# inferflow/inferflow

Measured on AMD Instinct MI355X. Metric: decode tokens/sec, Llama-2-7B Q4 batch=1 greedy (whole job), higher is better.
Workload: dtype i8 (Q8 activations x Q4_B32T1A weights, i32 dot, f32 scale, f16 I/O); 1 GPU; llama2_7b decode, Q4_B32T1A weights + F16 lm_head, F16 KV cache, batch 1 greedy, 16-token prompt, context 21..1851; parallelism=single, weights_bytes=4309647360

## Files before the change

### include/inferflow_amd.h

```cpp
#ifndef INFERFLOW_AMD_H_
#define INFERFLOW_AMD_H_

#include <stddef.h>
#include <stdint.h>

#ifdef __cplusplus
extern "C" {
#endif

typedef enum {
    IFA_F32 = 0, IFA_F16 = 1,
    IFA_Q8_B32T1 = 7, IFA_Q8_B32T2 = 8, IFA_Q6_B64T1 = 9, IFA_Q5_B64T1 = 10, IFA_Q5_B32T1 = 11,
    IFA_Q4_B16 = 12, IFA_Q4_B32T1A = 13, IFA_Q4_B32T1B = 14, IFA_Q4_B64T1 = 17, IFA_Q3H_B64T1 = 18,
    IFA_Q3_B32T1A = 19, IFA_Q3_B32T1B = 20, IFA_Q2_B32T1A = 21, IFA_Q2_B32T1B = 22
} ifa_dtype;

enum {
    IFA_OK = 0,
    IFA_ERR_ARG = -1,
    IFA_ERR_DTYPE = -2,
    IFA_ERR_HIP = -3,
    IFA_ERR_STATE = -4,
    IFA_ERR_NOMEM = -5
};
// ... 227 lines not shown
    int vocab_offset;
    int force_collectives;
} ifa_tp_topology;
int ifa_model_tp_decode(ifa_model *m, const ifa_tp_topology *topo, int first_token, int start_pos, int n_steps,
                        int *out_tokens_host, float *elapsed_ms);
int ifa_model_tp_prefill(ifa_model *m, const ifa_tp_topology *topo, const int *tokens_host, int n_tokens, int start_pos,
                         void *logits_shard_out_dev, int *next_token_host);
int ifa_model_tp_decode_batch(ifa_model *m, const ifa_tp_topology *topo, int n, const int *tokens_host, const int *positions_host,
                              const int *kv_slots_host, int *next_tokens_host, void *logits_shard_out_dev);
int ifa_model_get_tensor(ifa_model *m, int layer, int tensor_id, int *dtype, void **dptr, size_t *rows, size_t *cols);
int ifa_model_get_expert_tensor(ifa_model *m, int layer, int expert, int tensor_id, int *dtype, void **dptr, size_t *rows, size_t *cols);
int ifa_model_time_kernel(ifa_model *m, int which, int iters, float *avg_us);

int ifa_decode_route_plan(const int *facts, int n_facts, int *out, int n_out);
int ifa_model_decode_route(ifa_model *m, int *out, int n_out);

int ifa_prompt_route_plan(const int *facts, int n_facts, int *out, int n_out);
int ifa_batch_route_plan(const int *facts, int n_facts, int *out, int n_out);
int ifa_model_prompt_route(ifa_model *m, int *out, int n_out);

#ifdef __cplusplus
}
#endif
#endif
```

### inferflow_amd/_capi.py

```python
import ctypes as C
import os

_HERE = os.path.dirname(os.path.abspath(__file__))
_LIB_PATH = os.environ.get("IFA_LIB") or os.path.join(_HERE, "lib", "libinferflow_amd.so")
_lib = None


class IfaError(RuntimeError):
    def __init__(self, code, msg):
        super().__init__("inferflow_amd error %d: %s" % (code, msg))
        self.code = code


def library_path():
    return _LIB_PATH


def lib():
    global _lib
    if _lib is None:
        if not os.path.exists(_LIB_PATH):
            raise ImportError(
                "inferflow_amd: %s is missing -- run `python __graft_entry__.py build` "
                "(hipcc --offload-arch=gfx950); there is no CPU fallback" % _LIB_PATH)
# ... 96 lines not shown
    "ifa_model_decode_draft": (_i, [_vp, _i, _vp, _i, _vp, _vp]),
    "ifa_model_set_pool_excluded": (_i, [_vp, _vp, _i]),
    "ifa_model_decode_pool": (_i, [_vp, _i, _i, _i, _vp, _vp, _vp, _vp]),
    "ifa_model_decode_batch_pool": (_i, [_vp, _i, _vp, _vp, _vp, _vp, _i, _vp, _i, _vp, _vp, _vp]),
    "ifa_model_forward_pool": (_i, [_vp, _vp, _i, _i, _vp, _i, _vp, _vp, _vp, _vp]),
    "ifa_model_pool_lse": (_i, [_vp, _vp, _i, _vp]),
    "ifa_model_logit_state_reset": (_i, [_vp, _i, _vp, _i, _f, _f, _f, _vp, _vp, _i]),
    "ifa_model_logit_state_add": (_i, [_vp, _i, _vp, _vp]),
    "ifa_model_pool_adjust": (_i, [_vp, _i, _vp]),
    "ifa_model_forward_score": (_i, [_vp, _vp, _i, _i, _vp, _vp, _vp, _vp]),
    "ifa_model_get_buffer": (_i, [_vp, C.c_char_p, _i, C.POINTER(_vp), C.POINTER(_sz)]),
    "ifa_model_stream": (_vp, [_vp]),
    "ifa_model_time_kernel": (_i, [_vp, _i, _i, _vp]),
    "ifa_decode_route_plan": (_i, [_vp, _i, _vp, _i]),
    "ifa_model_decode_route": (_i, [_vp, _vp, _i]),
    "ifa_prompt_route_plan": (_i, [_vp, _i, _vp, _i]),
    "ifa_batch_route_plan": (_i, [_vp, _i, _vp, _i]),
    "ifa_model_prompt_route": (_i, [_vp, _vp, _i]),
    "ifa_model_set_stream": (_i, [_vp, _vp]),
    "ifa_model_tp_begin": (_i, [_vp, _i, _i]),
    "ifa_model_tp_begin_hidden": (_i, [_vp, _vp, _i]),
    "ifa_model_tp_hidden": (_i, [_vp, _vp]),
    "ifa_model_tp_attn": (_i, [_vp, _i, _vp]),
    "ifa_model_tp_post_attn": (_i, [_vp, _i, _vp]),
    "ifa_model_tp_ffn": (_i, [_vp, _i, _vp]),
    "ifa_model_tp_post_ffn": (_i, [_vp, _i, _vp]),
    "ifa_model_tp_logits": (_i, [_vp, _vp]),
    "ifa_model_tp_set_token": (_i, [_vp, _vp]),
    "ifa_comm_unique_id": (_i, [_vp]),
    "ifa_comm_init_rank": (_i, [_vp, _i, _i, _i, C.POINTER(_vp)]),
# ... 115 lines not shown
```

### inferflow_amd/csrc/ifa_decode_route.h

```cpp
#pragma once
#include <algorithm>
#include <cstddef>
#include <cstring>

static constexpr size_t IFA_LDS_LIMIT = 160 * 1024;

namespace ifa {
constexpr int DEC_ATTN_MAX_SPLITS = 32;
constexpr int DEC_PV_STAGE = 4096;

constexpr size_t dec_attn_scores_smem(int head_dim, bool q8) { return q8 ? 16 : (size_t)256 * (head_dim * 2 + 16); }
constexpr size_t dec_attn_pv_smem(int head_dim, int max_ctx, int nsplits = 8)
{
    const size_t nsplit = 256 / (head_dim / 8);
    const size_t chunk = (((size_t)max_ctx + nsplits - 1) / nsplits + 63) / 64 * 64;
    return 8 * 4 + nsplit * head_dim * 4 + (size_t)(DEC_PV_STAGE + 8) * 2 + chunk * 2 + 16;
}
constexpr size_t dec_attn_smem(int head_dim, int max_ctx, int ktile_rows = 0)
{
    const size_t nsplit = 256 / (head_dim / 8);
    return (size_t)head_dim * 3 * 2 + 16 * 4 + nsplit * head_dim * 4 + (size_t)ktile_rows * head_dim * 2 + (((size_t)max_ctx * 2 + 15) & ~(size_t)15) + 16;
}

inline bool dec_qkv_attn_ul_shape(int rw, int gk) { return (rw == 6 && gk == 8) || (rw == 3 && gk == 32); }
// ... 48 lines not shown
        r.kt = kt_fits;
        const bool unload = (f.attn_unload >= 1 && bucket == 256) || (f.attn_unload >= 2 && bucket == 128 && (r.kt || f.kv_q8));
        r.ul = unload && dec_qkv_attn_ul_shape(f.rw, f.gk);
        r.pb = (r.ul && bucket == 64) || (!f.kv_q8 && !r.kt) ? 256 : bucket;
        r.gk = f.gk; r.rw = f.rw;
    }
    if (r.kind != DEC_ROUTE_SPLIT) r.lds_attn = (int)dec_attn_smem(f.head_dim, f.max_ctx, r.kt ? r.pb : 0);
    if (!f.own_launches) {
        r.chain = (f.fuse_ffn && f.waits && f.num_cus <= f.visible_cus) ? std::min(f.fuse_ffn, 2) : 0;
        if (r.chain == 2 && (!f.have_attq || !f.attn_q8 || f.head_dim % 32 != 0)) r.chain = 1;
        r.chain = std::min(r.chain, f.chain_level);
    }
    return r;
}

}
```

### inferflow_amd/csrc/ifa_engine.hip

```cpp
#include <mutex>
#include <unordered_map>
#include "ifa_engine_state.h"

namespace ifa {

namespace {
struct SpaceBook {
    std::mutex mu;
    std::unordered_map<void *, size_t> live;
    long long live_bytes = 0, fail_at = 0;
};
SpaceBook &book() { static SpaceBook *b = new SpaceBook(); return *b; }

template <class Alloc> int space_alloc(const char *call, void **p, size_t bytes, Alloc alloc)
{
    SpaceBook &b = book();
    *p = nullptr;
    {
        std::lock_guard<std::mutex> g(b.mu);
        if (b.fail_at > 0 && --b.fail_at == 0)
            return ifa_fail(IFA_ERR_HIP, "%s(%zu bytes) failed: out of memory (simulated: ifa_debug_alloc_fail_at)", call, bytes);
    }
    const hipError_t e = alloc(p, bytes);
    if (e != hipSuccess) {
// ... 65 lines not shown

int perf_collect(ifa_model *m)
{
    if (m->perf_spans.empty()) return IFA_OK;
    IFA_HIP_CHECK(hipStreamSynchronize(m->stream));
    for (auto &r : m->perf_spans) {
        float ms = 0.0f;
        if (hipEventElapsedTime(&ms, r.e0, r.e1) == hipSuccess) m->perf_map[r.key] += ms;
        else (void)hipGetLastError();
        m->perf_pool.push_back(r.e0); m->perf_pool.push_back(r.e1);
    }
    m->perf_spans.clear();
    return IFA_OK;
}

void drop_graphs(ifa_model *m)
{
    if (m->tp_graph_exec) { (void)hipGraphExecDestroy(m->tp_graph_exec); m->tp_graph_exec = nullptr; }
    if (m->tp_graph) { (void)hipGraphDestroy(m->tp_graph); m->tp_graph = nullptr; }
    if (m->graph_exec) { (void)hipGraphExecDestroy(m->graph_exec); m->graph_exec = nullptr; }
    if (m->graph) { (void)hipGraphDestroy(m->graph); m->graph = nullptr; }
    if (m->graph_exec_n) { (void)hipGraphExecDestroy(m->graph_exec_n); m->graph_exec_n = nullptr; }
    if (m->graph_n) { (void)hipGraphDestroy(m->graph_n); m->graph_n = nullptr; }
    for (auto &sl : m->slots) {
        if (sl.exec) { (void)hipGraphExecDestroy(sl.exec); sl.exec = nullptr; }
        if (sl.graph) { (void)hipGraphDestroy(sl.graph); sl.graph = nullptr; }
    }
    for (auto &kv : m->batch_graphs) if (kv.second) (void)hipGraphExecDestroy(kv.second);
    m->batch_graphs.clear();
    for (auto &kv : m->draft_graphs) if (kv.second) (void)hipGraphExecDestroy(kv.second);
    m->draft_graphs.clear();
    sampled_drop_graphs(m);
}

int ensure_scratch(ifa_model *m, int T)
{
    if (T <= m->scratch_tokens) return IFA_OK;
    const ifa_model_config &c = m->cfg;
    const size_t D = c.dim, QD = (size_t)c.heads * c.head_dim, KVD = (size_t)c.kv_heads * c.head_dim, F = c.ffn;
    size_t maxcols = std::max(std::max(D, QD), F);
    Scratch n;
    int rc;
// ... 359 lines not shown
    IFA_HIP_CHECK(hipStreamSynchronize(m->stream));
    return IFA_OK;
}

int ifa_model_select_kv(ifa_model *m, int slot)
{
    IFA_REQUIRE(m && m->finalized, "ifa_model_select_kv: model not finalized");
    if (m->slots.empty()) m->slots.resize(1);
    IFA_REQUIRE(slot >= 0 && slot < (int)m->slots.size(), "ifa_model_select_kv: slot %d of %zu", slot, m->slots.size());
    if (slot == m->cur_slot) return IFA_OK;
    if (m->tp_graph_exec) { (void)hipGraphExecDestroy(m->tp_graph_exec); m->tp_graph_exec = nullptr; }
    if (m->tp_graph) { (void)hipGraphDestroy(m->tp_graph); m->tp_graph = nullptr; }
    ifa_model::KvSlot &out = m->slots[(size_t)m->cur_slot], &in = m->slots[(size_t)slot];
    out.k.clear(); out.v.clear();
    for (Layer &L : m->layers) { out.k.push_back(std::move(L.kcache)); out.v.push_back(std::move(L.vcache)); }
    out.graph = m->graph; out.exec = m->graph_exec;
    if (m->graph_exec_n) { (void)hipGraphExecDestroy(m->graph_exec_n); m->graph_exec_n = nullptr; }
    if (m->graph_n) { (void)hipGraphDestroy(m->graph_n); m->graph_n = nullptr; }
    for (size_t l = 0; l < m->layers.size(); l++) { m->layers[l].kcache = std::move(in.k[l]); m->layers[l].vcache = std::move(in.v[l]); }
    m->graph = in.graph; m->graph_exec = in.exec;
    in.k.clear(); in.v.clear(); in.graph = nullptr; in.exec = nullptr;
    m->cur_slot = slot;
    return IFA_OK;
}

int ifa_model_set_option(ifa_model *m, const char *name, int value)
{
    IFA_REQUIRE(m && name, "ifa_model_set_option: null pointer");
    if (strcmp(name, "pool_lse") == 0) { m->opt_pool_lse = value != 0; return IFA_OK; }
    struct { const char *n; int *p; } opts[] = {
        {"fused", &m->opt_fused}, {"graph", &m->opt_graph}, {"rpw_qkv", &m->opt_rpw_qkv}, {"rpw_wo", &m->opt_rpw_wo},
        {"rpw_ffn", &m->opt_rpw_ffn}, {"rpw_w2", &m->opt_rpw_w2}, {"rpw_lm", &m->opt_rpw_lm}, {"trace", &m->opt_trace},
        {"bench_mode", &m->opt_bench_mode}, {"touch_stride", &m->opt_touch_stride}, {"attn_split_ctx", &m->opt_attn_split_ctx}, {"batch_graph", &m->opt_batch_graph}, {"gemm_rows", &m->opt_gemm_rows}, {"batch_fused", &m->opt_batch_fused}, {"rows_mo", &m->opt_rows_mo}, {"debug_mo_alloc_fail", &m->opt_debug_mo_alloc_fail}, {"rows_kparts", &m->opt_rows_kparts}, {"prefill_chunk", &m->opt_prefill_chunk}, {"prefill_big_min", &m->opt_prefill_big_min}, {"prefill_mid", &m->opt_prefill_mid}, {"prefill_mid_max", &m->opt_prefill_mid_max}, {"prefill_res_mid", &m->opt_prefill_res_mid}, {"gemm_splitk", &m->opt_gemm_splitk}, {"moe_singles", &m->opt_moe_singles}, {"moe_overlap", &m->opt_moe_overlap}, {"prefill_big", &m->opt_prefill_big}, {"moe_router_fused", &m->opt_moe_router_fused}, {"tp_fuse_add", &m->opt_tp_fuse_add}, {"attn_q8", &m->opt_attn_q8}, {"attn_kt", &m->opt_attn_kt}, {"fuse_attn", &m->opt_fuse_attn}, {"fuse_ffn", &m->opt_fuse_ffn}, {"attn_post_as_residual", &m->opt_attn_post_as_residual}, {"chain_late_w2", &m->opt_chain_late_w2}, {"exact_order", &m->opt_exact_order}, {"perf_stat", &m->opt_perf_stat}, {"attn_nsplits", &m->opt_attn_nsplits}, {"attn_unload", &m->opt_attn_unload}, {"q3h_native", &m->opt_q3h_native}, {"fuse_attn_timeout_us", &m->opt_fuse_attn_timeout_us}, {"step_tail", &m->opt_step_tail}, {"graph_steps", &m->opt_graph_steps}, {"moe_device", &m->opt_moe_device}, 
        
        {"debug_layers", &m->opt_debug_layers}, {"debug_layer0", &m->opt_debug_layer0}, {"debug_hidden_in", &m->opt_debug_hidden_in}};
    for (auto &o : opts)
// ... 37 lines not shown
    IFA_REQUIRE(m, "ifa_model_fused_supported: null model");
    std::string w;
    bool ok = fused_supported(m, &w);
    if (why && why_len) { strncpy(why, w.c_str(), why_len - 1); why[why_len - 1] = 0; }
    return ok ? 1 : 0;
}

int ifa_decode_route_plan(const int *facts, int n_facts, int *out, int n_out)
{
    IFA_REQUIRE(facts && out && n_facts == DEC_ROUTE_N_FACTS && n_out >= DEC_ROUTE_N_OUT, "ifa_decode_route_plan: %d facts, %d outputs expected", DEC_ROUTE_N_FACTS, DEC_ROUTE_N_OUT);
    DecRouteFacts f;
    memcpy(&f, facts, sizeof(f));
    IFA_REQUIRE(f.head_dim >= 8 && f.max_ctx >= 1, "ifa_decode_route_plan: head_dim %d, max_ctx %d", f.head_dim, f.max_ctx);
    const DecRoute r = plan_decode_route(f);
    memcpy(out, &r, sizeof(r));
    return IFA_OK;
}

int ifa_model_decode_route(ifa_model *m, int *out, int n_out)
{
    IFA_REQUIRE(m && out && n_out >= DEC_ROUTE_N_OUT + 3, "ifa_model_decode_route: %d outputs expected", DEC_ROUTE_N_OUT + 3);
    memcpy(out, &m->route, sizeof(m->route));
    out[DEC_ROUTE_N_OUT] = num_cus(); out[DEC_ROUTE_N_OUT + 1] = visible_cus(); out[DEC_ROUTE_N_OUT + 2] = waits_enabled() ? 1 : 0;
    return IFA_OK;
}

int ifa_prompt_route_plan(const int *facts, int n_facts, int *out, int n_out)
{
    IFA_REQUIRE(facts && out && n_facts == PROMPT_ROUTE_N_FACTS && n_out >= PROMPT_ROUTE_N_OUT, "ifa_prompt_route_plan: %d facts, %d outputs expected", PROMPT_ROUTE_N_FACTS, PROMPT_ROUTE_N_OUT);
    PromptRouteFacts f;
// ... 98 lines not shown
```

### inferflow_amd/csrc/ifa_engine_decode.hip

```cpp
#include "ifa_engine_state.h"

namespace ifae {


__global__ void __launch_bounds__(256) k_touch(const uint8_t *__restrict__ p, size_t bytes, size_t stride, int *sink)
{
    size_t i = ((size_t)blockIdx.x * blockDim.x + threadIdx.x) * stride;
    int acc = 0;
    for (; i < bytes; i += (size_t)gridDim.x * blockDim.x * stride) acc += *reinterpret_cast<const int *>(p + i);
    if (acc == 0x7FFFFFFF) *sink = acc;
}

static long long *g_trace_ptr = nullptr;

bool fused_ok(const Tensor &t, bool long_rows)
{
    if (!t.present()) return false;
    if (fused_int8(t.dtype)) return t.tiled && (long_rows ? dec_gemv_supported_long(t.dtype, t.cols) : dec_gemv_supported(t.dtype, t.cols));
    return dec_gemv_h_supported(t.dtype, t.cols) && (long_rows || t.cols <= 8192);
}

template <int EPI, int NORM>
static int launch_dec_gemv(int w_dtype, const DecGemvParams &P, int wgs_per_cu_opt, hipStream_t s)
{
// ... 136 lines not shown
{
    const ifa_model_config &c = m->cfg;
    DecRouteFacts f;
    f.head_dim = c.head_dim; f.heads = c.heads; f.kv_heads = c.kv_heads; f.max_ctx = c.max_ctx; f.kv_q8 = c.kv_dtype == Q8_B32T2;
    f.reach = reach;
    f.attn_split_ctx = m->opt_attn_split_ctx; f.attn_nsplits = m->opt_attn_nsplits; f.attn_kt = m->opt_attn_kt; f.attn_unload = m->opt_attn_unload;
    f.fuse_attn = m->opt_fuse_attn; f.fuse_ffn = m->opt_fuse_ffn; f.attn_q8 = m->opt_attn_q8;
    f.waits = waits_enabled(); f.num_cus = num_cus(); f.visible_cus = visible_cus();
    f.have_attq = m->attq ? 1 : 0; f.own_launches = own_launches;
    f.tail_layers_ok = f.fuse_attn && f.waits;
    for (int l = 0; f.tail_layers_ok && l < c.layers; l++) if (!qkv_attn_layer_ok(m, l, &f.gk, &f.rw)) f.tail_layers_ok = 0;
    f.chain_level = (f.fuse_ffn && f.waits && !own_launches) ? chain_level(m) : 0;
    return f;
}

int decode_route_ready(ifa_model *m, int reach, bool own_launches)
{
    const ifa_model_config &c = m->cfg;
    const DecRoute route = plan_decode_route(route_facts(m, reach, own_launches));
    m->route_reach = reach;
    if (!(route == m->route)) { m->route = route; drop_graphs(m); }
    if (route.kind == DEC_ROUTE_FUSED_TAIL && !m->qa_gran) {
        const size_t n = (size_t)c.layers * (size_t)(c.heads + 2 * c.kv_heads) * c.head_dim;
        DevBuf<unsigned long long> gran; DevBuf<unsigned> call, err;
        int rc;
        if ((rc = gran.alloc(n)) || (rc = call.alloc(4)) || (rc = err.alloc(4))) return rc;
        IFA_HIP_CHECK(hipMemsetAsync(gran, 0, n * 8, m->stream));
        IFA_HIP_CHECK(hipMemsetAsync(call, 0, 16, m->stream));
        IFA_HIP_CHECK(hipMemsetAsync(err, 0, 16, m->stream));
        m->qa_gran = std::move(gran); m->qa_call = std::move(call); m->qa_err = std::move(err);
        IFA_HIP_CHECK(hipStreamSynchronize(m->stream));
    }
    if (route.chain && !m->ch_gran) {
        const size_t n = (size_t)c.layers * (size_t)(c.dim + (int)m->layers[0].t[T_W1].rows);
        DevBuf<uint32_t> gran, flags; DevBuf<unsigned> call, err;
        int rc;
        if ((rc = gran.alloc(n)) || (rc = flags.alloc((size_t)c.layers * 2 * 1024))) return rc;
        IFA_HIP_CHECK(hipMemsetAsync(gran, 0, n * 4, m->stream));
        IFA_HIP_CHECK(hipMemsetAsync(flags, 0, (size_t)c.layers * 2 * 1024 * 4, m->stream));
        if (!m->qa_call) { if ((rc = call.alloc(4))) return rc; IFA_HIP_CHECK(hipMemsetAsync(call, 0, 16, m->stream)); }
        if (!m->qa_err) { if ((rc = err.alloc(4))) return rc; IFA_HIP_CHECK(hipMemsetAsync(err, 0, 16, m->stream)); }
        m->ch_gran = std::move(gran); m->ch_flags = std::move(flags);
        if (call) m->qa_call = std::move(call);
        if (err) m->qa_err = std::move(err);
        IFA_HIP_CHECK(hipStreamSynchronize(m->stream));
    }
    return IFA_OK;
}

void qkv_params(ifa_model *m, int l, const half_t *x, DecGemvParams &P)
{
    const ifa_model_config &c = m->cfg;
    Layer &L = m->layers[(size_t)l];
    memset(&P, 0, sizeof(P));
    P.x = x; P.norm_w = (const half_t *)L.t[T_ATTN_NORM].data; P.norm_b = (const half_t *)L.t[T_ATTN_NORM_B].data;
    P.multi_base = c.attn_norm_base; P.eps = c.eps; P.cols = c.dim; P.nblk = c.dim / 32;
    if (c.parallel_attn) P.xn_out = m->xn;
    const int ids[3] = {T_WQ, T_WK, T_WV}; const int bids[3] = {T_WQ_B, T_WK_B, T_WV_B};
    const size_t QDd = (size_t)c.heads * c.head_dim, KVDd = (size_t)c.kv_heads * c.head_dim;
    half_t *outs[3] = {m->dqkv, m->dqkv + QDd, m->dqkv + QDd + KVDd};
    for (int i = 0; i < 3; i++) {
        P.W0[i] = wbytes(L.t[ids[i]]); P.b0[i] = (const half_t *)L.t[bids[i]].data;
// ... 413 lines not shown
{
    int rc = IFA_OK;
    IFA_HIP_CHECK(hipStreamSynchronize(m->stream));
    IFA_HIP_CHECK(hipStreamBeginCapture(m->stream, hipStreamCaptureModeThreadLocal));
    for (int i = 0; i < n && !rc; i++) rc = enqueue_fused_step(m);
    hipGraph_t gph = nullptr;
    hipError_t e = hipStreamEndCapture(m->stream, &gph);
    if (rc) { if (gph) (void)hipGraphDestroy(gph); return rc; }
    if (e != hipSuccess) return ifa_fail(IFA_ERR_HIP, "hipStreamEndCapture: %s", hipGetErrorString(e));
    if (*graph) (void)hipGraphDestroy(*graph);
    *graph = gph;
    IFA_HIP_CHECK(hipGraphInstantiate(exec, gph, nullptr, nullptr, 0));
    return IFA_OK;
}

int decode_impl(ifa_model *m, int first_token, int start_pos, int n_steps, int *out_tokens_host, float *elapsed_ms, bool prepare_only,
                const SampledCall *sc)
{
    IFA_REQUIRE(m && m->finalized, "ifa_model_decode: model not finalized");
    IFA_REQUIRE(n_steps > 0 && n_steps <= ifa_model::RING, "ifa_model_decode: n_steps %d (max %d per call)", n_steps, ifa_model::RING);
    IFA_REQUIRE(start_pos >= 0 && start_pos + n_steps <= m->cfg.max_ctx, "ifa_model_decode: positions [%d,%d) exceed max_ctx %d",
                start_pos, start_pos + n_steps, m->cfg.max_ctx);
    IFA_REQUIRE(m->g[T_EMBD].present() && m->g[T_LM_HEAD].present(), "ifa_model_decode: embeddings / lm_head missing (pipeline stage worker)");
    IFA_HIP_CHECK(hipSetDevice(m->cfg.device));
    std::string why;
    const bool exact = m->opt_exact_order != 0;
    if (exact || !m->opt_fused || m->opt_perf_stat || !fused_supported(m, &why)) {
        if (prepare_only) return IFA_OK;
        int tok = first_token;
        for (int i = 0; i < n_steps; i++) {
            int nt = 0;
            int rc = exact ? forward_exact(m, tok, start_pos + i, nullptr, &nt) : forward_ops(m, &tok, 1, start_pos + i, nullptr, &nt);
            if (rc) return rc;
            if (out_tokens_host) out_tokens_host[i] = nt;
            tok = nt;
        }
        if (elapsed_ms) *elapsed_ms = -1.0f;
        return IFA_OK;
    }
    static const bool trace_host = getenv("IFA_TRACE_DECODE") != nullptr;
    const auto th0 = std::chrono::steady_clock::now();
    auto th = [&](const char *what) {
        if (trace_host) fprintf(stderr, "decode-host %-28s %8.1f us\n", what, std::chrono::duration<double, std::micro>(std::chrono::steady_clock::now() - th0).count());
    };
    int rc = ensure_scratch(m, 1);
    if (rc) return rc;
    if (m->opt_q3h_native && (rc = ensure_q3hn(m))) return rc;
    hipStream_t s = m->stream;
    if ((rc = decode_route_ready(m, start_pos + n_steps))) return rc;
    const bool waits_on = m->route.kind == DEC_ROUTE_FUSED_TAIL || m->route.chain;
    if ((rc = step_tail_ready(m))) return rc;
    m->host_pinned[0] = first_token; m->host_pinned[1] = start_pos; m->host_pinned[2] = 0;
    IFA_HIP_CHECK(hipMemcpyAsync(m->state, m->host_pinned, 3 * sizeof(int), hipMemcpyHostToDevice, s));
    if (waits_on) {
        m->qa_calls = (m->qa_calls % 4000u) + 1u;
        m->host_pinned[6] = (int)m->qa_calls;
        IFA_HIP_CHECK(hipMemcpyAsync(m->qa_call, m->host_pinned + 6, sizeof(int), hipMemcpyHostToDevice, s));
    }
    hipGraphExec_t samp_exec = nullptr;
    if (sc) {
        if ((rc = sampled_prepare(m, *sc))) return rc;
        if (m->opt_graph && (rc = sampled_graph(m, &samp_exec))) return rc;
        if ((rc = sampled_begin(m, *sc))) return rc;
    }
    if (!sc && m->opt_graph && !m->graph_exec && (rc = capture_steps(m, 1, &m->graph, &m->graph_exec))) return rc;
    const int S = m->opt_graph_steps;
    if (!sc && m->opt_graph && S > 1 && n_steps >= S && (!m->graph_exec_n || m->graph_n_steps != S)) {
        if (m->graph_exec_n) { (void)hipGraphExecDestroy(m->graph_exec_n); m->graph_exec_n = nullptr; }
        if (m->graph_n) { (void)hipGraphDestroy(m->graph_n); m->graph_n = nullptr; }
        if ((rc = capture_steps(m, S, &m->graph_n, &m->graph_exec_n))) return rc;
        m->graph_n_steps = S;
    }
    if (prepare_only) return IFA_OK;
    th("state copies enqueued");
    hipEvent_t e0 = nullptr, e1 = nullptr;
    if (elapsed_ms) { IFA_HIP_CHECK(hipEventCreate(&e0)); IFA_HIP_CHECK(hipEventCreate(&e1)); IFA_HIP_CHECK(hipEventRecord(e0, s)); }
    th("events created, first recorded");
    if (!sc && m->st_on && (rc = launch_gather(m))) return rc;
    for (int i = 0; i < n_steps;) {
        if (sc) {
            if (samp_exec) IFA_HIP_CHECK(hipGraphLaunch(samp_exec, s));
            else if ((rc = enqueue_fused_step(m, STEP_TAIL_SAMPLED))) return rc;
            i++;
            continue;
        }
        if (m->opt_graph && m->graph_exec_n && m->graph_n_steps == S && S > 1 && n_steps - i >= S) { IFA_HIP_CHECK(hipGraphLaunch(m->graph_exec_n, s)); i += S; continue; }
        if (m->opt_graph) IFA_HIP_CHECK(hipGraphLaunch(m->graph_exec, s));
        else if ((rc = enqueue_fused_step(m))) return rc;
        i++;
    }
    th("steps enqueued");
    if (elapsed_ms) IFA_HIP_CHECK(hipEventRecord(e1, s));
    if (!sc && (rc = pool_enqueue(m, m->logits, 1))) return rc;
    if (sc && (rc = sampled_copy_back(m))) return rc;
    IFA_HIP_CHECK(hipMemcpyAsync(m->host_pinned + 8, m->state + 8, sizeof(int) * (size_t)n_steps, hipMemcpyDeviceToHost, s));
    int *qerr = m->host_pinned + 8 + ifa_model::RING;
    qerr[0] = 0;
    if (waits_on) IFA_HIP_CHECK(hipMemcpyAsync(qerr, m->qa_err, 4, hipMemcpyDeviceToHost, s));
    th("copies back enqueued");
    IFA_HIP_CHECK(hipStreamSynchronize(s));
    th("stream synchronised");
    if ((rc = qa_err_check(m, qerr[0])) || (sc && (rc = sampled_finish(m, *sc)))) {
// ... 75 lines not shown
```

### inferflow_amd/csrc/ifa_engine_state.h

```cpp
#pragma once
#include <chrono>
#include <cstdlib>
#include <cstring>
#include <map>
#include <string>
#include <type_traits>
#include <vector>
#include "ifa_host.h"
#include "ifa_buf_hip.h"
#include "ifa_decode_kernels.h"
#include "ifa_decode_attn.h"
#include "ifa_decode_gemv.h"
#include "ifa_moe.h"
#include "ifa_gemm_rows_mfma.h"
#include "ifa_gemm_big.h"
#include "ifa_decode_lmhead_tail.h"
#include "ifa_decode_singles.h"
#include "ifa_decode_qkv_attn.h"
#include "ifa_decode_chain.h"
#include "ifa_prompt_route.h"

using namespace ifa;

namespace ifae {
// ... 54 lines not shown
    ifa_model_config cfg;
    std::vector<Layer> layers;
    Tensor g[10];
    hipStream_t stream = nullptr;
    hipStream_t side_stream = nullptr; Event ev_fork, ev_join; int opt_moe_overlap = 1;
    bool own_stream = true;
    bool finalized = false;
    int opt_moe_device = 1;
    DevBuf<int> state;
    DevBuf<float> rope_tab;
    DevBuf<long long> trace;
    int opt_trace = 0, opt_bench_mode = 0, opt_touch_stride = 65536;
    PinBuf<int> host_pinned;
    int scratch_tokens = 0;
    size_t kv_row_bytes = 0;
    hipGraph_t graph = nullptr;
    hipGraphExec_t graph_exec = nullptr;
    hipGraph_t graph_n = nullptr; hipGraphExec_t graph_exec_n = nullptr; int graph_n_steps = 0, opt_graph_steps = 1;
    struct PendingAdd { const half_t *x = nullptr, *add = nullptr, *bias = nullptr; half_t *out = nullptr; bool on = false; } pend;
    int opt_tp_fuse_add = 1;
    DevPin<void> batch_tab;
    std::map<int, hipGraphExec_t> batch_graphs;
    std::map<int, hipGraphExec_t> draft_graphs;
    DecAttnSplitWs attn_ws = {nullptr, nullptr, nullptr, 8};
    DevBuf<half_t> attn_ws_S; DevBuf<float> attn_ws_lmax, attn_ws_opart;
    int opt_attn_unload = 1;
    int opt_attn_nsplits = 0;
    DecRoute route; int route_reach = 256;
    PromptRoute prompt_route;
    int opt_fuse_attn = 1, opt_fuse_attn_timeout_us = 20000;
    DevBuf<unsigned long long> qa_gran;
    DevBuf<unsigned> qa_call, qa_err; unsigned qa_calls = 0;
    int opt_fuse_ffn = 0, opt_chain_late_w2 = 0;
    int opt_q3h_native = 0;
    int opt_perf_stat = 0;
    struct PerfSpanRec { int key; hipEvent_t e0, e1; };
    std::vector<PerfSpanRec> perf_spans;
    std::vector<hipEvent_t> perf_pool;
    std::map<int, float> perf_map;
    int opt_exact_order = 0;
    DevBuf<float> exact_rope_tab;
    DevBuf<uint32_t> ch_gran, ch_flags;
    int opt_step_tail = 1, st_on = 0;
    DevBuf<unsigned long long> st_keys; DevBuf<unsigned> st_counter;
    int opt_attn_kt = 1;
    int opt_attn_split_ctx = -1, opt_batch_graph = 0, opt_gemm_rows = 1, opt_batch_fused = 1, opt_moe_router_fused = 1, opt_prefill_big = 1, opt_rows_mo = 1, opt_moe_singles = 1;
    struct KvSlot { std::vector<DevBuf<void>> k, v; hipGraph_t graph = nullptr; hipGraphExec_t exec = nullptr; };
    std::vector<KvSlot> slots;
    int cur_slot = 0;
    int opt_attn_q8 = 1;
    DevBuf<half_t> tp_a, tp_f, tp_hid, tp_logits;
    DevBuf<float> tp_best, tp_gather;
    DevBuf<int> tp_tok;
    hipGraph_t tp_graph = nullptr;
    hipGraphExec_t tp_graph_exec = nullptr;
    struct TpKey {
        unsigned long long tp = 0, world = 0; int tp_size = 0, stage = 0, n_stages = 0, prev = 0, next = 0, src = 0, voff = 0, force = 0, fuse = 0, slot = 0, oneshot = 0;
        bool operator==(const TpKey &o) const { return tp == o.tp && world == o.world && tp_size == o.tp_size && stage == o.stage && n_stages == o.n_stages
                && prev == o.prev && next == o.next && src == o.src && voff == o.voff && force == o.force && fuse == o.fuse && slot == o.slot
                && oneshot == o.oneshot; }
    } tp_key;
    const ifa_tp_topology *topo = nullptr;
// ... 117 lines not shown
template <class F>
static int attn_dispatch(int head_dim, bool q8, F &&f)
{
    using std::integral_constant;
    switch (head_dim) {
    case 32: return q8 ? f(integral_constant<int, 32>{}, std::true_type{}) : f(integral_constant<int, 32>{}, std::false_type{});
    case 64: return q8 ? f(integral_constant<int, 64>{}, std::true_type{}) : f(integral_constant<int, 64>{}, std::false_type{});
    case 96: return q8 ? f(integral_constant<int, 96>{}, std::true_type{}) : f(integral_constant<int, 96>{}, std::false_type{});
    case 128: return q8 ? f(integral_constant<int, 128>{}, std::true_type{}) : f(integral_constant<int, 128>{}, std::false_type{});
    case 48: if (!q8) return f(integral_constant<int, 48>{}, std::false_type{}); break;
    case 80: if (!q8) return f(integral_constant<int, 80>{}, std::false_type{}); break;
    }
    return ifa_fail(IFA_ERR_ARG, "fused attention: head_dim %d with %s cache", head_dim, q8 ? "a Q8" : "an F16");
}

void drop_graphs(ifa_model *m);
int perf_begin(ifa_model *m, int key);
void perf_end(ifa_model *m, int idx);
int perf_collect(ifa_model *m);
struct PerfSpan {
    ifa_model *m; int idx;
    PerfSpan(ifa_model *mm, int key, bool on = true) : m(mm), idx(on ? perf_begin(mm, key) : -1) {}
    ~PerfSpan() { done(); }
    void done() { if (idx >= 0) { perf_end(m, idx); idx = -1; } }
};
void *kv_ptr(ifa_model *m, size_t layer, int slot, bool is_v);
int kv_copy_table(ifa_model *m, int a, int b);
int ensure_mo(ifa_model *m);
int ensure_mo_build(ifa_model *m);
int ensure_x32(ifa_model *m);
int ensure_q3hn(ifa_model *m);
int ensure_scratch(ifa_model *m, int T);
bool fused_ok(const Tensor &t, bool long_rows);
int lmhead_grid(const DecLmHeadParams &P, int wgs_per_cu_opt);
int launch_lmhead(const DecLmHeadParams &P, int norm, int wgs_per_cu_opt, hipStream_t s, const DecStepTail *Z = nullptr);
bool has_post_norms(const ifa_model *m);
bool fused_supported(const ifa_model *m, std::string *why);
int sep_norm(ifa_model *m, const half_t *x, const Tensor &w, const Tensor &b, half_t *dst);
void attn_params(ifa_model *m, int l, DecAttnParams &A);
int decode_route_ready(ifa_model *m, int reach, bool own_launches = false);
void qkv_params(ifa_model *m, int l, const half_t *x, DecGemvParams &P);
int launch_qkv_attn(ifa_model *m, int l, const half_t *x, unsigned tag_add = 0);
int launch_qkv(ifa_model *m, int l, const half_t *x);
int launch_attn(ifa_model *m, int l);
int launch_wo(ifa_model *m, int l, const half_t *x, half_t *partial = nullptr);
void moe_params(ifa_model *m, Layer &L, DecGemvParams &P, int slot, int tab_off);
int launch_ffn13(ifa_model *m, int l, int moe_slot = -1, const half_t *x_layer = nullptr, int moe_nslots = 1);
int launch_w2(ifa_model *m, int l, half_t *xnext, half_t *partial = nullptr, int moe_slot = -1, bool moe_last = false,
                     const half_t *residual2 = nullptr, int moe_t1_slot = 0);
int launch_chain(ifa_model *m, int l, const half_t *x, half_t *xnext, unsigned tag_add = 0);
bool step_tail_ok(const ifa_model *m);
DecLmHeadParams lm_params(ifa_model *m, const half_t *x, half_t *logits_out);
int step_tail_ready(ifa_model *m);
int launch_lm_tail(ifa_model *m, const half_t *x);
int launch_gather(ifa_model *m);
// ... 52 lines not shown
```

### inferflow_amd/worker.py

```python
import ctypes as C

import numpy as np

from . import _capi, dtypes as dt
from ._capi import ModelConfig, check, lib

T_EMBD, T_OUT_NORM, T_OUT_NORM_B, T_LM_HEAD = 0, 1, 2, 3
T_ATTN_NORM, T_ATTN_NORM_B, T_WQ, T_WK, T_WV, T_WO = 10, 11, 12, 13, 14, 15
T_FFN_NORM, T_FFN_NORM_B, T_W1, T_W2, T_W3, T_MOE_GATE = 16, 17, 18, 19, 20, 21
T_WQ_B, T_WK_B, T_WV_B, T_WO_B, T_W1_B, T_W2_B, T_W3_B = 22, 23, 24, 25, 26, 27, 28
T_ATTN_POST_NORM, T_ATTN_POST_NORM_B, T_FFN_POST_NORM, T_FFN_POST_NORM_B = 29, 30, 31, 32

_DEFAULTS = dict(norm_kind=0, act_kind=0, is_glu=1, rope_order=2, use_alibi=0, parallel_attn=0, share_input=0,
                 rope_theta=10000.0, partial_rotary=1.0, kq_scale=1.0, eps=1e-5, kv_dtype=dt.F16,
                 full_quant_gemv=1, experts=0, moe_top_k=0, moe_norm_topk=1, tp_rank=0, tp_size=1, device=0,
                 attn_norm_base=0.0, ffn_norm_base=0.0, out_norm_base=0.0, attn_out_scale=1.0, ffn_out_scale=1.0, out_scale=1.0,
                 embd_scale=0.0)


class DecodeWorker:
    def __init__(self, **kw):
        cfg = ModelConfig()
        vals = dict(_DEFAULTS)
        vals.update(kw)
# ... 193 lines not shown
    def time_kernel(self, which, iters=200):
        us = C.c_float(0)
        check(lib().ifa_model_time_kernel(self._h, which, iters, C.byref(us)))
        return us.value

    ROUTE_FIELDS = ("kind", "nsplits", "pb", "kt", "ul", "gk", "rw", "chain", "split_threshold", "split", "lds_attn", "lds_scores", "lds_pv",
                    "error", "num_cus", "visible_cus", "waits")
    ROUTE_KINDS = ("one_workgroup", "split", "fused_tail")

    def decode_route(self):
        out = (C.c_int * len(self.ROUTE_FIELDS))()
        check(lib().ifa_model_decode_route(self._h, out, len(out)))
        d = dict(zip(self.ROUTE_FIELDS, out))
        d["kind"] = self.ROUTE_KINDS[d["kind"]]
        return d

    PROMPT_ROUTE_FIELDS = ("kind", "first_pass", "norm_fused", "res_mid") + tuple(
        p + "_" + k for p in ("qkv", "wo", "w13", "w2") for k in ("kernel", "src", "mo", "no_waits")) + ("need_mo", "need_x32")
    PROMPT_ROUTE_KINDS = ("exact", "op_by_op", "rows", "mid", "big")

    def prompt_route(self):
        out = (C.c_int * len(self.PROMPT_ROUTE_FIELDS))()
        check(lib().ifa_model_prompt_route(self._h, out, len(out)))
        d = dict(zip(self.PROMPT_ROUTE_FIELDS, out))
        d["kind"] = self.PROMPT_ROUTE_KINDS[d["kind"]]
        return d

    def get_tensor_host(self, layer, tid):
        d, p, r, c = C.c_int(), C.c_void_p(), C.c_size_t(), C.c_size_t()
        rc = lib().ifa_model_get_tensor(self._h, layer, tid, C.byref(d), C.byref(p), C.byref(r), C.byref(c))
# ... 303 lines not shown
```

Before: 621.9 tokens/s.

## Segment decode calls by context reach and cache one step graph per route

Decode previously planned a single route from the final context reach and captured one step graph for the whole call. It now splits the call's positions at fixed edges (64, 128, the split threshold, 8192) and plans a route per segment, so early short-context steps can use the route best suited to their actual reach. Each distinct route gets its own captured step graph, held in a small LRU cache per KV slot. The cost is extra graph captures and memory for several graphs, plus new bookkeeping on slot switches and route changes.

```diff
diff --git a/include/inferflow_amd.h b/include/inferflow_amd.h
--- a/include/inferflow_amd.h
+++ b/include/inferflow_amd.h
@@ -265,6 +265,8 @@
 
 int ifa_decode_route_plan(const int *facts, int n_facts, int *out, int n_out);
 int ifa_model_decode_route(ifa_model *m, int *out, int n_out);
+int ifa_decode_segments_plan(const int *facts, int n_facts, int start_pos, int n_steps, int *out, int n_out);
+int ifa_model_decode_segments(ifa_model *m, int *out, int n_out);
 
 int ifa_prompt_route_plan(const int *facts, int n_facts, int *out, int n_out);
 int ifa_batch_route_plan(const int *facts, int n_facts, int *out, int n_out);
diff --git a/inferflow_amd/_capi.py b/inferflow_amd/_capi.py
--- a/inferflow_amd/_capi.py
+++ b/inferflow_amd/_capi.py
@@ -134,6 +134,8 @@
     "ifa_model_time_kernel": (_i, [_vp, _i, _i, _vp]),
     "ifa_decode_route_plan": (_i, [_vp, _i, _vp, _i]),
     "ifa_model_decode_route": (_i, [_vp, _vp, _i]),
+    "ifa_decode_segments_plan": (_i, [_vp, _i, _i, _i, _vp, _i]),
+    "ifa_model_decode_segments": (_i, [_vp, _vp, _i]),
     "ifa_prompt_route_plan": (_i, [_vp, _i, _vp, _i]),
     "ifa_batch_route_plan": (_i, [_vp, _i, _vp, _i]),
     "ifa_model_prompt_route": (_i, [_vp, _vp, _i]),
diff --git a/inferflow_amd/csrc/ifa_decode_route.h b/inferflow_amd/csrc/ifa_decode_route.h
--- a/inferflow_amd/csrc/ifa_decode_route.h
+++ b/inferflow_amd/csrc/ifa_decode_route.h
@@ -86,4 +86,27 @@
     return r;
 }
 
+struct DecSegment { int first_step = 0, n_steps = 0; DecRoute route; };
+constexpr int DEC_ROUTE_MAX_SEGMENTS = 5;
+
+inline int plan_decode_segments(DecRouteFacts f, int start_pos, int n_steps, DecSegment *out)
+{
+    const int end = start_pos + n_steps;
+    f.reach = end;
+    if (f.own_launches) { out[0].first_step = 0; out[0].n_steps = n_steps; out[0].route = plan_decode_route(f); return 1; }
+    int edges[5] = {64, 128, plan_decode_route(f).split_threshold, 8192, end};
+    std::sort(edges, edges + 5);
+    int n = 0, lo = start_pos;
+    for (int e : edges) {
+        const int reach = std::min(e, end);
+        if (reach <= lo) continue;
+        f.reach = reach;
+        const DecRoute r = plan_decode_route(f);
+        if (n > 0 && out[n - 1].route == r) out[n - 1].n_steps += reach - lo;
+        else { out[n].first_step = lo - start_pos; out[n].n_steps = reach - lo; out[n].route = r; n++; }
+        lo = reach;
+    }
+    return n;
 }
+
+}
diff --git a/inferflow_amd/csrc/ifa_engine.hip b/inferflow_amd/csrc/ifa_engine.hip
--- a/inferflow_amd/csrc/ifa_engine.hip
+++ b/inferflow_amd/csrc/ifa_engine.hip
@@ -103,18 +103,25 @@
     return IFA_OK;
 }
 
-void drop_graphs(ifa_model *m)
+static void drop_step_graphs(std::vector<ifa_model::StepGraph> &steps)
+{
+    for (auto &g : steps) {
+        if (g.exec) (void)hipGraphExecDestroy(g.exec);
+        if (g.graph) (void)hipGraphDestroy(g.graph);
+    }
+    steps.clear();
+}
+
+void drop_graphs(ifa_model *m, bool keep_steps)
 {
     if (m->tp_graph_exec) { (void)hipGraphExecDestroy(m->tp_graph_exec); m->tp_graph_exec = nullptr; }
     if (m->tp_graph) { (void)hipGraphDestroy(m->tp_graph); m->tp_graph = nullptr; }
-    if (m->graph_exec) { (void)hipGraphExecDestroy(m->graph_exec); m->graph_exec = nullptr; }
-    if (m->graph) { (void)hipGraphDestroy(m->graph); m->graph = nullptr; }
+    if (!keep_steps) {
+        drop_step_graphs(m->step_graphs);
+        for (auto &sl : m->slots) drop_step_graphs(sl.steps);
+    }
     if (m->graph_exec_n) { (void)hipGraphExecDestroy(m->graph_exec_n); m->graph_exec_n = nullptr; }
     if (m->graph_n) { (void)hipGraphDestroy(m->graph_n); m->graph_n = nullptr; }
-    for (auto &sl : m->slots) {
-        if (sl.exec) { (void)hipGraphExecDestroy(sl.exec); sl.exec = nullptr; }
-        if (sl.graph) { (void)hipGraphDestroy(sl.graph); sl.graph = nullptr; }
-    }
     for (auto &kv : m->batch_graphs) if (kv.second) (void)hipGraphExecDestroy(kv.second);
     m->batch_graphs.clear();
     for (auto &kv : m->draft_graphs) if (kv.second) (void)hipGraphExecDestroy(kv.second);
@@ -504,12 +511,12 @@
     ifa_model::KvSlot &out = m->slots[(size_t)m->cur_slot], &in = m->slots[(size_t)slot];
     out.k.clear(); out.v.clear();
     for (Layer &L : m->layers) { out.k.push_back(std::move(L.kcache)); out.v.push_back(std::move(L.vcache)); }
-    out.graph = m->graph; out.exec = m->graph_exec;
+    out.steps = std::move(m->step_graphs);
     if (m->graph_exec_n) { (void)hipGraphExecDestroy(m->graph_exec_n); m->graph_exec_n = nullptr; }
     if (m->graph_n) { (void)hipGraphDestroy(m->graph_n); m->graph_n = nullptr; }
     for (size_t l = 0; l < m->layers.size(); l++) { m->layers[l].kcache = std::move(in.k[l]); m->layers[l].vcache = std::move(in.v[l]); }
-    m->graph = in.graph; m->graph_exec = in.exec;
-    in.k.clear(); in.v.clear(); in.graph = nullptr; in.exec = nullptr;
+    m->step_graphs = std::move(in.steps);
+    in.k.clear(); in.v.clear(); in.steps.clear();
     m->cur_slot = slot;
     return IFA_OK;
 }
@@ -577,6 +584,35 @@
     IFA_REQUIRE(f.head_dim >= 8 && f.max_ctx >= 1, "ifa_decode_route_plan: head_dim %d, max_ctx %d", f.head_dim, f.max_ctx);
     const DecRoute r = plan_decode_route(f);
     memcpy(out, &r, sizeof(r));
+    return IFA_OK;
+}
+
+int ifa_decode_segments_plan(const int *facts, int n_facts, int start_pos, int n_steps, int *out, int n_out)
+{
+    constexpr int per = 2 + DEC_ROUTE_N_OUT;
+    IFA_REQUIRE(facts && out && n_facts == DEC_ROUTE_N_FACTS && n_out >= 1 + DEC_ROUTE_MAX_SEGMENTS * per, "ifa_decode_segments_plan: %d facts, %d outputs expected", DEC_ROUTE_N_FACTS, 1 + DEC_ROUTE_MAX_SEGMENTS * per);
+    DecRouteFacts f;
+    memcpy(&f, facts, sizeof(f));
+    IFA_REQUIRE(f.head_dim >= 8 && f.max_ctx >= 1, "ifa_decode_segments_plan: head_dim %d, max_ctx %d", f.head_dim, f.max_ctx);
+    IFA_REQUIRE(start_pos >= 0 && n_steps > 0, "ifa_decode_segments_plan: start_pos %d, n_steps %d", start_pos, n_steps);
+    DecSegment segs[DEC_ROUTE_MAX_SEGMENTS];
+    out[0] = plan_decode_segments(f, start_pos, n_steps, segs);
+    for (int i = 0; i < out[0]; i++) {
+        out[1 + i * per] = segs[i].first_step; out[2 + i * per] = segs[i].n_steps;
+        memcpy(out + 3 + i * per, &segs[i].route, sizeof(DecRoute));
+    }
+    return IFA_OK;
+}
+
+int ifa_model_decode_segments(ifa_model *m, int *out, int n_out)
+{
+    constexpr int per = 2 + DEC_ROUTE_N_OUT;
+    IFA_REQUIRE(m && out && n_out >= 2 + DEC_ROUTE_MAX_SEGMENTS * per, "ifa_model_decode_segments: %d outputs expected", 2 + DEC_ROUTE_MAX_SEGMENTS * per);
+    out[0] = m->last_n_segs; out[1] = m->last_captures;
+    for (int i = 0; i < m->last_n_segs; i++) {
+        out[2 + i * per] = m->last_start_pos + m->last_segs[i].first_step; out[3 + i * per] = m->last_segs[i].n_steps;
+        memcpy(out + 4 + i * per, &m->last_segs[i].route, sizeof(DecRoute));
+    }
     return IFA_OK;
 }
 
diff --git a/inferflow_amd/csrc/ifa_engine_decode.hip b/inferflow_amd/csrc/ifa_engine_decode.hip
--- a/inferflow_amd/csrc/ifa_engine_decode.hip
+++ b/inferflow_amd/csrc/ifa_engine_decode.hip
@@ -174,13 +174,10 @@
     return f;
 }
 
-int decode_route_ready(ifa_model *m, int reach, bool own_launches)
-{
-    const ifa_model_config &c = m->cfg;
-    const DecRoute route = plan_decode_route(route_facts(m, reach, own_launches));
-    m->route_reach = reach;
-    if (!(route == m->route)) { m->route = route; drop_graphs(m); }
-    if (route.kind == DEC_ROUTE_FUSED_TAIL && !m->qa_gran) {
+static int route_buffers_ready(ifa_model *m, bool tail, bool chain)
+{
+    const ifa_model_config &c = m->cfg;
+    if (tail && !m->qa_gran) {
         const size_t n = (size_t)c.layers * (size_t)(c.heads + 2 * c.kv_heads) * c.head_dim;
         DevBuf<unsigned long long> gran; DevBuf<unsigned> call, err;
         int rc;
@@ -191,7 +188,7 @@
         m->qa_gran = std::move(gran); m->qa_call = std::move(call); m->qa_err = std::move(err);
         IFA_HIP_CHECK(hipStreamSynchronize(m->stream));
     }
-    if (route.chain && !m->ch_gran) {
+    if (chain && !m->ch_gran) {
         const size_t n = (size_t)c.layers * (size_t)(c.dim + (int)m->layers[0].t[T_W1].rows);
         DevBuf<uint32_t> gran, flags; DevBuf<unsigned> call, err;
         int rc;
@@ -206,6 +203,16 @@
         IFA_HIP_CHECK(hipStreamSynchronize(m->stream));
     }
     return IFA_OK;
+}
+
+int decode_route_ready(ifa_model *m, int reach, bool own_launches, DecRouteFacts *facts_out)
+{
+    const DecRouteFacts facts = route_facts(m, reach, own_launches);
+    const DecRoute route = plan_decode_route(facts);
+    if (facts_out) *facts_out = facts;
+    m->route_reach = reach;
+    if (!(route == m->route)) { m->route = route; drop_graphs(m, true); }
+    return route_buffers_ready(m, route.kind == DEC_ROUTE_FUSED_TAIL, route.chain != 0);
 }
 
 void qkv_params(ifa_model *m, int l, const half_t *x, DecGemvParams &P)
@@ -649,6 +656,31 @@
     return IFA_OK;
 }
 
+static int step_graph_ready(ifa_model *m, const DecRoute &route, hipGraphExec_t *exec)
+{
+    static_assert((size_t)DEC_ROUTE_MAX_SEGMENTS < ifa_model::STEP_GRAPHS, "a call's segments must fit the slot's cache of captured steps");
+    const unsigned long long now = ++m->step_clock;
+    for (auto &g : m->step_graphs)
+        if (g.route == route) { g.used = now; *exec = g.exec; return IFA_OK; }
+    ifa_model::StepGraph g;
+    g.route = route; g.used = now;
+    const DecRoute call_route = m->route;
+    m->route = route;
+    const int rc = capture_steps(m, 1, &g.graph, &g.exec);
+    m->route = call_route;
+    if (rc) { if (g.graph) (void)hipGraphDestroy(g.graph); return rc; }
+    if (m->step_graphs.size() >= ifa_model::STEP_GRAPHS) {
+        auto lru = std::min_element(m->step_graphs.begin(), m->step_graphs.end(), [](const ifa_model::StepGraph &a, const ifa_model::StepGraph &b) { return a.used < b.used; });
+        if (lru->exec) (void)hipGraphExecDestroy(lru->exec);
+        if (lru->graph) (void)hipGraphDestroy(lru->graph);
+        m->step_graphs.erase(lru);
+    }
+    m->step_graphs.push_back(g);
+    m->last_captures++;
+    *exec = g.exec;
+    return IFA_OK;
+}
+
 int decode_impl(ifa_model *m, int first_token, int start_pos, int n_steps, int *out_tokens_host, float *elapsed_ms, bool prepare_only,
                 const SampledCall *sc)
 {
@@ -658,6 +690,7 @@
                 start_pos, start_pos + n_steps, m->cfg.max_ctx);
     IFA_REQUIRE(m->g[T_EMBD].present() && m->g[T_LM_HEAD].present(), "ifa_model_decode: embeddings / lm_head missing (pipeline stage worker)");
     IFA_HIP_CHECK(hipSetDevice(m->cfg.device));
+    m->last_n_segs = 0; m->last_captures = 0; m->last_start_pos = start_pos;
     std::string why;
     const bool exact = m->opt_exact_order != 0;
     if (exact || !m->opt_fused || m->opt_perf_stat || !fused_supported(m, &why)) {
@@ -682,8 +715,18 @@
     if (rc) return rc;
     if (m->opt_q3h_native && (rc = ensure_q3hn(m))) return rc;
     hipStream_t s = m->stream;
-    if ((rc = decode_route_ready(m, start_pos + n_steps))) return rc;
-    const bool waits_on = m->route.kind == DEC_ROUTE_FUSED_TAIL || m->route.chain;
+    DecRouteFacts facts;
+    if ((rc = decode_route_ready(m, start_pos + n_steps, false, &facts))) return rc;
+    const bool step_graphs = !sc && m->opt_graph;
+    DecSegment *segs = m->last_segs;
+    int n_segs = 1;
+    if (step_graphs && m->opt_graph_steps <= 1 && m->route.kind != DEC_ROUTE_SPLIT) n_segs = plan_decode_segments(facts, start_pos, n_steps, segs);
+    else { segs[0].first_step = 0; segs[0].n_steps = n_steps; segs[0].route = m->route; }
+    m->last_n_segs = n_segs;
+    bool any_tail = false, any_chain = false;
+    for (int i = 0; i < n_segs; i++) { any_tail |= segs[i].route.kind == DEC_ROUTE_FUSED_TAIL; any_chain |= segs[i].route.chain != 0; }
+    if ((rc = route_buffers_ready(m, any_tail, any_chain))) return rc;
+    const bool waits_on = any_tail || any_chain;
     if ((rc = step_tail_ready(m))) return rc;
     m->host_pinned[0] = first_token; m->host_pinned[1] = start_pos; m->host_pinned[2] = 0;
     IFA_HIP_CHECK(hipMemcpyAsync(m->state, m->host_pinned, 3 * sizeof(int), hipMemcpyHostToDevice, s));
@@ -698,7 +741,8 @@
         if (m->opt_graph && (rc = sampled_graph(m, &samp_exec))) return rc;
         if ((rc = sampled_begin(m, *sc))) return rc;
     }
-    if (!sc && m->opt_graph && !m->graph_exec && (rc = capture_steps(m, 1, &m->graph, &m->graph_exec))) return rc;
+    hipGraphExec_t seg_exec[DEC_ROUTE_MAX_SEGMENTS] = {};
+    for (int i = 0; step_graphs && i < n_segs; i++) if ((rc = step_graph_ready(m, segs[i].route, &seg_exec[i]))) return rc;
     const int S = m->opt_graph_steps;
     if (!sc && m->opt_graph && S > 1 && n_steps >= S && (!m->graph_exec_n || m->graph_n_steps != S)) {
         if (m->graph_exec_n) { (void)hipGraphExecDestroy(m->graph_exec_n); m->graph_exec_n = nullptr; }
@@ -712,7 +756,7 @@
     if (elapsed_ms) { IFA_HIP_CHECK(hipEventCreate(&e0)); IFA_HIP_CHECK(hipEventCreate(&e1)); IFA_HIP_CHECK(hipEventRecord(e0, s)); }
     th("events created, first recorded");
     if (!sc && m->st_on && (rc = launch_gather(m))) return rc;
-    for (int i = 0; i < n_steps;) {
+    for (int i = 0, seg = 0; i < n_steps;) {
         if (sc) {
             if (samp_exec) IFA_HIP_CHECK(hipGraphLaunch(samp_exec, s));
             else if ((rc = enqueue_fused_step(m, STEP_TAIL_SAMPLED))) return rc;
@@ -720,7 +764,10 @@
             continue;
         }
         if (m->opt_graph && m->graph_exec_n && m->graph_n_steps == S && S > 1 && n_steps - i >= S) { IFA_HIP_CHECK(hipGraphLaunch(m->graph_exec_n, s)); i += S; continue; }
-        if (m->opt_graph) IFA_HIP_CHECK(hipGraphLaunch(m->graph_exec, s));
+        if (m->opt_graph) {
+            while (i >= segs[seg].first_step + segs[seg].n_steps) seg++;
+            IFA_HIP_CHECK(hipGraphLaunch(seg_exec[seg], s));
+        }
         else if ((rc = enqueue_fused_step(m))) return rc;
         i++;
     }
diff --git a/inferflow_amd/csrc/ifa_engine_state.h b/inferflow_amd/csrc/ifa_engine_state.h
--- a/inferflow_amd/csrc/ifa_engine_state.h
+++ b/inferflow_amd/csrc/ifa_engine_state.h
@@ -92,8 +92,10 @@
     PinBuf<int> host_pinned;
     int scratch_tokens = 0;
     size_t kv_row_bytes = 0;
-    hipGraph_t graph = nullptr;
-    hipGraphExec_t graph_exec = nullptr;
+    struct StepGraph { DecRoute route; hipGraph_t graph = nullptr; hipGraphExec_t exec = nullptr; unsigned long long used = 0; };
+    static constexpr size_t STEP_GRAPHS = 6;
+    std::vector<StepGraph> step_graphs; unsigned long long step_clock = 0;
+    DecSegment last_segs[DEC_ROUTE_MAX_SEGMENTS]; int last_n_segs = 0, last_start_pos = 0, last_captures = 0;
     hipGraph_t graph_n = nullptr; hipGraphExec_t graph_exec_n = nullptr; int graph_n_steps = 0, opt_graph_steps = 1;
     struct PendingAdd { const half_t *x = nullptr, *add = nullptr, *bias = nullptr; half_t *out = nullptr; bool on = false; } pend;
     int opt_tp_fuse_add = 1;
@@ -123,7 +125,7 @@
     DevBuf<unsigned long long> st_keys; DevBuf<unsigned> st_counter;
     int opt_attn_kt = 1;
     int opt_attn_split_ctx = -1, opt_batch_graph = 0, opt_gemm_rows = 1, opt_batch_fused = 1, opt_moe_router_fused = 1, opt_prefill_big = 1, opt_rows_mo = 1, opt_moe_singles = 1;
-    struct KvSlot { std::vector<DevBuf<void>> k, v; hipGraph_t graph = nullptr; hipGraphExec_t exec = nullptr; };
+    struct KvSlot { std::vector<DevBuf<void>> k, v; std::vector<StepGraph> steps; };
     std::vector<KvSlot> slots;
     int cur_slot = 0;
     int opt_attn_q8 = 1;
@@ -271,7 +273,7 @@
     return ifa_fail(IFA_ERR_ARG, "fused attention: head_dim %d with %s cache", head_dim, q8 ? "a Q8" : "an F16");
 }
 
-void drop_graphs(ifa_model *m);
+void drop_graphs(ifa_model *m, bool keep_steps = false);
 int perf_begin(ifa_model *m, int key);
 void perf_end(ifa_model *m, int idx);
 int perf_collect(ifa_model *m);
@@ -295,7 +297,7 @@
 bool fused_supported(const ifa_model *m, std::string *why);
 int sep_norm(ifa_model *m, const half_t *x, const Tensor &w, const Tensor &b, half_t *dst);
 void attn_params(ifa_model *m, int l, DecAttnParams &A);
-int decode_route_ready(ifa_model *m, int reach, bool own_launches = false);
+int decode_route_ready(ifa_model *m, int reach, bool own_launches = false, DecRouteFacts *facts_out = nullptr);
 void qkv_params(ifa_model *m, int l, const half_t *x, DecGemvParams &P);
 int launch_qkv_attn(ifa_model *m, int l, const half_t *x, unsigned tag_add = 0);
 int launch_qkv(ifa_model *m, int l, const half_t *x);
diff --git a/inferflow_amd/worker.py b/inferflow_amd/worker.py
--- a/inferflow_amd/worker.py
+++ b/inferflow_amd/worker.py
@@ -231,6 +231,19 @@
         d = dict(zip(self.ROUTE_FIELDS, out))
         d["kind"] = self.ROUTE_KINDS[d["kind"]]
         return d
+
+    def decode_segments(self):
+        names = self.ROUTE_FIELDS[:14]
+        per = 2 + len(names)
+        out = (C.c_int * (2 + 5 * per))()
+        check(lib().ifa_model_decode_segments(self._h, out, len(out)))
+        segs = []
+        for i in range(out[0]):
+            row = out[2 + i * per:2 + (i + 1) * per]
+            d = dict(zip(names, row[2:]), pos=row[0], steps=row[1])
+            d["kind"] = self.ROUTE_KINDS[d["kind"]]
+            segs.append(d)
+        return segs, out[1]
 
     PROMPT_ROUTE_FIELDS = ("kind", "first_pass", "norm_fused", "res_mid") + tuple(
         p + "_" + k for p in ("qkv", "wo", "w13", "w2") for k in ("kernel", "src", "mo", "no_waits")) + ("need_mo", "need_x32")
```

Result: no change. 621.7 tokens/s (median of 2 runs) (-0.0%).
